# sebasv/lp

Hardware: AMD Instinct MI355X
Metric: IPM iterations/sec, dense 4096x8192 fp64 LP (higher is better)
Workload: dtype f64; 1 GPU; C3: random dense planted LP m=4096 n=8192 fp64, one independent LP per GPU (seed = rank), reference default options, A resident in HBM; m=4096, n=8192

## Files before the change

### lp_amd/csrc/kernels_adat.hip

```cpp
#include "gemm_tile.hpp"

namespace lpipm {

__device__ __forceinline__ int xcd_remap(int b, int n) {
    const int xcd = b & 7, q = n >> 3, r = n & 7;
    return (xcd < r ? xcd * (q + 1) : r * (q + 1) + (xcd - r) * q) + (b >> 3);
}

typedef unsigned int u4v __attribute__((ext_vector_type(4)));
typedef unsigned int u2v __attribute__((ext_vector_type(2)));
__device__ __forceinline__ __amdgpu_buffer_rsrc_t make_rsrc(const void* base, unsigned bytes) {
    return __builtin_amdgcn_make_buffer_rsrc(const_cast<void*>(base), 0, (int)bytes, 0x00020000);
}
__device__ __forceinline__ d2 buf_load_d2(__amdgpu_buffer_rsrc_t r, unsigned voff, unsigned soff) {
    return __builtin_bit_cast(d2, __builtin_amdgcn_raw_buffer_load_b128(r, (int)voff, (int)soff, 0));
}
__device__ __forceinline__ double buf_load_d(__amdgpu_buffer_rsrc_t r, unsigned voff, unsigned soff) {
    return __builtin_bit_cast(double, __builtin_amdgcn_raw_buffer_load_b64(r, (int)voff, (int)soff, 0));
}
__device__ __forceinline__ void buf_store_d(__amdgpu_buffer_rsrc_t r, unsigned voff, unsigned soff, double v) {
    __builtin_amdgcn_raw_buffer_store_b64(__builtin_bit_cast(u2v, v), r, (int)voff, (int)soff, 0);
}
template <int AUX>
__device__ __forceinline__ void buf_store_d_aux(__amdgpu_buffer_rsrc_t r, unsigned voff, unsigned soff, double v) {
    __builtin_amdgcn_raw_buffer_store_b64(__builtin_bit_cast(u2v, v), r, (int)voff, (int)soff, AUX);
}
template <int AUX>
__device__ __forceinline__ void buf_store_d2_aux(__amdgpu_buffer_rsrc_t r, unsigned voff, unsigned soff, d2 v) {
    __builtin_amdgcn_raw_buffer_store_b128(__builtin_bit_cast(u4v, v), r, (int)voff, (int)soff, AUX);
}
template <int AUX>
__device__ __forceinline__ d2 buf_load_d2_aux(__amdgpu_buffer_rsrc_t r, unsigned voff, unsigned soff) {
    return __builtin_bit_cast(d2, __builtin_amdgcn_raw_buffer_load_b128(r, (int)voff, (int)soff, AUX));
}

__device__ __forceinline__ int diag_pattern(int wr, int wc) {
    const int d = 2 * wc - 4 * wr;
    return d < 0 ? 0 : (d == 0 ? 1 : (d == 2 ? 2 : 3));
}
__device__ __forceinline__ void wave_part(int wave, int& wr, int& wc) {
    wr = (0x4B >> wave) & 1;
    wc = (0x7E84 >> (2 * wave)) & 3;
}
__device__ __forceinline__ constexpr int diag_group(int mi, int nj) {
    return nj > mi ? 1 : (2 + nj > mi ? 2 : 3);
}

template <typename F> __device__ __forceinline__ void diag_dispatch(int pat, F&& f) {
    if (pat == 0) f.template operator()<0>();
    else if (pat == 1) f.template operator()<1>();
    else if (pat == 2) f.template operator()<2>();
    else f.template operator()<3>();
}

template <int PAT = 0, typename FL, typename TC>
__device__ __forceinline__ void tile_pass_w8(double (*ldsA)[TILE][LDS_STRIDE], double (*ldsB)[TILE][LDS_STRIDE],
                                             __amdgpu_buffer_rsrc_t Pr, unsigned p64, __amdgpu_buffer_rsrc_t Qr, unsigned q64,
                                             __amdgpu_buffer_rsrc_t Sr, unsigned offP, unsigned offQ, unsigned offS,
                                             int kb, int ke, d4 (&acc)[4][2],
                                             int srow, int scol, int wr, int wc, int fr, int fq, int kc, FL&& flush,
                                             TC&& touch) {
    d2 sa[2], sb[2], sv;
    auto gload = [&](int kt) {
        const unsigned ko = (unsigned)kt * (unsigned)(BK * sizeof(double));
        sv = buf_load_d2(Sr, offS, ko);
        sa[0] = buf_load_d2(Pr, offP, ko);
        sa[1] = buf_load_d2(Pr, offP, ko + p64);
        sb[0] = buf_load_d2(Qr, offQ, ko);
        sb[1] = buf_load_d2(Qr, offQ, ko + q64);
    };
    auto lstore = [&](int buf) {
#pragma unroll
        for (int r = 0; r < 2; ++r) *(d2*)&ldsA[buf][srow + 64 * r][lds_wcol(srow, scol)] = sa[r];
#pragma unroll
        for (int r = 0; r < 2; ++r) *(d2*)&ldsB[buf][srow + 64 * r][lds_wcol(srow, scol)] = sb[r] * sv;
    };
    auto mfma_ktile = [&](int cur) {
        if constexpr (PAT < 3) {
#pragma unroll
            for (int round = 0; round < 2; ++round) {
                d2 a[4] = {}, b[2] = {};
                if (round == 0) __builtin_amdgcn_s_setprio(0);
#pragma unroll
                for (int mi = 0; mi < 4; ++mi)
                    if (diag_group(mi, 0) > PAT) a[mi] = *(const d2*)&ldsA[cur][wr * 64 + mi * 16 + fr][round * 8 + lds_rq(fr, fq)];
#pragma unroll
                for (int nj = 0; nj < 2; ++nj)
                    if (diag_group(3, nj) > PAT) b[nj] = *(const d2*)&ldsB[cur][wc * 32 + nj * 16 + fr][round * 8 + lds_rq(fr, fq)];
#pragma unroll
                for (int t = 0; t < 2; ++t)
#pragma unroll
                    for (int mi = 0; mi < 4; ++mi)
#pragma unroll
                        for (int nj = 0; nj < 2; ++nj)
                            if (diag_group(mi, nj) > PAT)
                                acc[mi][nj] = __builtin_amdgcn_mfma_f64_16x16x4f64(a[mi][t], b[nj][t], acc[mi][nj], 0, 0, 0);
            }
        }
        __builtin_amdgcn_s_setprio(2);
    };
    gload(kb);
    lstore(0);
    __syncthreads();
    int cur = 0, kt = kb;
    bool first = true;
    while (kt < ke) {
        int ce = ke;
        if (kc > 0) { const int e = (kt / kc + 1) * kc; ce = e < ke ? e : ke; }
        for (; kt < ce - 1; ++kt) {
            gload(kt + 1);
            mfma_ktile(cur);
            lstore(cur ^ 1);
            __syncthreads();
            cur ^= 1;
        }
        const bool more = ce < ke;
        unsigned pf0 = 0, pf1 = 0;
        touch(first, pf0, pf1);
        if (more) gload(ce);
        mfma_ktile(cur);
        if (more) lstore(cur ^ 1);
        asm volatile("" :: "v"(pf0), "v"(pf1));
        flush(first, !more);
        if (more) acc_clear(acc);
        first = false;
        __syncthreads();
        cur ^= 1;
        kt = ce;
    }
    __builtin_amdgcn_s_setprio(0);
}

struct Round2K {
    const double* A; long long lda;
    const double* s;
    double* C; long long ldc;
    int KT;
    int ntiles;
    const int2* tile_list;
    int diag_pad_from;
    double* ws;
    int nwg;
    unsigned int* sk_claim;
    int kc;
    int sk;
    double* C2;
    BatchK bk;
    long long astride;
};
__device__ __forceinline__ Round2K batch_shift(const Round2K& p0) {
    Round2K p = p0;
    p.A = (const double*)((const char*)p0.A + batch_lp(p0.bk) * p0.astride);
    p.s = batch_ptr(p0.s, p0.bk);
    p.C = batch_ptr(p0.C, p0.bk); p.ws = batch_ptr(p0.ws, p0.bk); p.sk_claim = batch_ptr(p0.sk_claim, p0.bk);
    p.C2 = batch_ptr(p0.C2, p0.bk);
    return p;
}
__global__ __launch_bounds__(512) __attribute__((amdgpu_waves_per_eu(4, 4))) void gemm_nt_streamk_w8_kernel(const Round2K p0) {
    if (batch_done(p0.bk)) return;
    const Round2K p = batch_shift(p0);
    __shared__ __attribute__((aligned(16))) double ldsA[2][TILE][LDS_STRIDE];
    __shared__ __attribute__((aligned(16))) double ldsB[2][TILE][LDS_STRIDE];
    const int tid = threadIdx.x, lane = tid & 63, wave = __builtin_amdgcn_readfirstlane(tid >> 6);
    int wr, wc;
    wave_part(wave, wr, wc);
    const int fr = lane & 15, fq = lane >> 4;
    const int srow = tid >> 3, scol = (tid & 7) * 2;
    const int g = p.bk.xcd_major ? (int)blockIdx.y : xcd_remap(blockIdx.x, gridDim.x);
    const int KT = p.KT;
    const int ntiles_dp = (p.ntiles / p.nwg) * p.nwg;
    const unsigned rowC = (unsigned)(p.ldc * (long long)sizeof(double));
    const unsigned offC = (unsigned)(wr * 64 + fq) * rowC + (unsigned)((wc * 32 + fr) * sizeof(double));
    auto c_rsrc = [&](int ti, int tj) { return make_rsrc(p.C + (long long)(ti * TILE) * p.ldc + tj * TILE, (unsigned)TILE * rowC); };
    auto store_tile = [&](const d4 (&acc)[4][2], int ti, int tj) {
        double* cb = p.C + (long long)(ti * TILE + wr * 64 + fq) * p.ldc + (tj * TILE + wc * 32 + fr);
        tile_store<4, 2>(cb, p.ldc, acc, 1.0, 0.0, p.diag_pad_from >= 0 && ti == tj, ti * TILE + wr * 64 + fq,
                         p.diag_pad_from, fr, fq, wc * 32 - wr * 64);
    };
    auto add_tile = [&](const d4 (&acc)[4][2], int ti, int tj, bool final_copy) {
        const __amdgpu_buffer_rsrc_t cr = c_rsrc(ti, tj);
        const __amdgpu_buffer_rsrc_t cr2 = make_rsrc((final_copy ? p.C2 : p.C) + (long long)(ti * TILE) * p.ldc + tj * TILE, (unsigned)TILE * rowC);
#pragma unroll
        for (int h = 0; h < 2; ++h) {
            double cv[2][4][2];
#pragma unroll
            for (int m2 = 0; m2 < 2; ++m2)
#pragma unroll
                for (int r = 0; r < 4; ++r)
#pragma unroll
                    for (int nj = 0; nj < 2; ++nj)
                        cv[m2][r][nj] = buf_load_d(cr, offC, (unsigned)((2 * h + m2) * 16 + 4 * r) * rowC + nj * 128);
#pragma unroll
            for (int m2 = 0; m2 < 2; ++m2)
#pragma unroll
                for (int r = 0; r < 4; ++r)
#pragma unroll
                    for (int nj = 0; nj < 2; ++nj)
                    {
                        const double v = cv[m2][r][nj] + acc[2 * h + m2][nj][r];
                        buf_store_d(cr, offC, (unsigned)((2 * h + m2) * 16 + 4 * r) * rowC + nj * 128, v);
                        if (final_copy) buf_store_d(cr2, offC, (unsigned)((2 * h + m2) * 16 + 4 * r) * rowC + nj * 128, v);
                    }
        }
    };
    auto touch_tile = [&](int ti, int tj, unsigned& pf0, unsigned& pf1) {
        const __amdgpu_buffer_rsrc_t cr = c_rsrc(ti, tj);
        const unsigned off = (unsigned)(wr * 64 + lane) * rowC + (unsigned)(wc * 32 * sizeof(double));
        pf0 = __builtin_amdgcn_raw_buffer_load_b32(cr, (int)off, 0, 0);
        pf1 = __builtin_amdgcn_raw_buffer_load_b32(cr, (int)off, 128, 0);
    };
    const unsigned rowA = (unsigned)(p.lda * (long long)sizeof(double));
    const unsigned offP = (unsigned)srow * rowA + (unsigned)(scol * sizeof(double));
    const unsigned offS = (unsigned)(scol * sizeof(double));
    const unsigned p64 = 64u * rowA;
    auto a_rsrc = [&](int t) { return make_rsrc(p.A + (long long)(t * TILE) * p.lda, (unsigned)TILE * rowA); };
    const __amdgpu_buffer_rsrc_t Sr = make_rsrc(p.s, (unsigned)KT * (unsigned)(BK * sizeof(double)));
    for (int tile = g; tile < ntiles_dp; tile += p.nwg) {
        const int ti = p.tile_list[tile].x, tj = p.tile_list[tile].y;
        d4 acc[4][2];
        acc_clear(acc);
        tile_pass_w8(ldsA, ldsB, a_rsrc(ti), p64, a_rsrc(tj), p64, Sr, offP, offP, offS, 0, KT, acc, srow, scol, wr, wc, fr, fq,
                            p.kc, [&](bool first, bool last) {
                                if (first) store_tile(acc, ti, tj); else add_tile(acc, ti, tj, last && p.C2 != nullptr);
                            },
                            [&](bool first, unsigned& pf0, unsigned& pf1) { if (!first) touch_tile(ti, tj, pf0, pf1); });
    }
    if (ntiles_dp == p.ntiles) return;
    __shared__ int s_claim;
    const int ch_tiles = p.sk;
    const int cpt = (KT + ch_tiles - 1) / ch_tiles;
    const int nchunks = (p.ntiles - ntiles_dp) * cpt;
    for (;;) {
        if (tid == 0) s_claim = (int)atomicAdd(p.sk_claim, 1u);
        __syncthreads();
        const int ch = __builtin_amdgcn_readfirstlane(s_claim);
        __syncthreads();
        if (ch >= nchunks) break;
        const int nrem = p.ntiles - ntiles_dp;
        const int q = ch / nrem, rt = ch - q * nrem;
        const int kb = q * ch_tiles, ke = kb + ch_tiles < KT ? kb + ch_tiles : KT;
        const int ti = p.tile_list[ntiles_dp + rt].x, tj = p.tile_list[ntiles_dp + rt].y;
        d4 acc[4][2];
        acc_clear(acc);
        tile_pass_w8(ldsA, ldsB, a_rsrc(ti), p64, a_rsrc(tj), p64, Sr, offP, offP, offS, kb, ke, acc, srow, scol, wr, wc, fr, fq,
                            0, [&](bool, bool) {
            if (cpt == 1) { store_tile(acc, ti, tj); return; }
            const __amdgpu_buffer_rsrc_t wr_ = make_rsrc(p.ws + ((long long)rt * cpt + q) * (TILE * TILE), (unsigned)(TILE * TILE * sizeof(double)));
            const unsigned offW = (unsigned)(((wr * 64 + fq) * TILE + wc * 32 + fr) * sizeof(double));
#pragma unroll
            for (int mi = 0; mi < 4; ++mi)
#pragma unroll
                for (int r = 0; r < 4; ++r)
#pragma unroll
                    for (int nj = 0; nj < 2; ++nj)
                        buf_store_d(wr_, offW, (unsigned)(((mi * 16 + 4 * r) * TILE + nj * 16) * sizeof(double)), acc[mi][nj][r]);
        }, [](bool, unsigned&, unsigned&) {});
    }
}

constexpr int FIX_SPLIT = 16;
__global__ __launch_bounds__(256) void gemm_nt_fixup_kernel(const Round2K p0) {
    if (batch_done(p0.bk)) return;
    const Round2K p = batch_shift(p0);
    const int ntiles_dp = (p.ntiles / p.nwg) * p.nwg;
    const int bx = p.bk.xcd_major ? (int)blockIdx.y : (int)blockIdx.x;
    const int rt = bx / FIX_SPLIT, part = bx % FIX_SPLIT;
    const int cpt = (p.KT + p.sk - 1) / p.sk;
    const int ti = p.tile_list[ntiles_dp + rt].x, tj = p.tile_list[ntiles_dp + rt].y;
    constexpr int PER = TILE * TILE / FIX_SPLIT;
    const double* slab0 = p.ws + (long long)rt * cpt * (TILE * TILE);
    for (int e = part * PER + threadIdx.x * 2; e < (part + 1) * PER; e += 512) {
        d2 sum = *(const d2*)(slab0 + e);
        for (int q = 1; q < cpt; ++q) sum += *(const d2*)(slab0 + (long long)q * (TILE * TILE) + e);
        const int r = e / TILE, c = e - r * TILE;
        const int row = ti * TILE + r, col = tj * TILE + c;
        double* cp = p.C + (long long)row * p.ldc + col;
        d2 v = sum;
        if (p.diag_pad_from >= 0) {
            if (row == col && row >= p.diag_pad_from) v[0] = 1.0;
            if (row == col + 1 && row >= p.diag_pad_from) v[1] = 1.0;
        }
        *(d2*)cp = v;
        if (p.C2) *(d2*)(p.C2 + (long long)row * p.ldc + col) = v;
    }
}

constexpr int AUX_SC1 = 16;
struct UnitsK {
    const double* A; long long lda;
    const double* s;
    double* C; long long ldc;
    double* C2;
    int KT, kc, cpt;
    int nbig, ks;
    int ntiles;
    const int2* tile_list;
    const int2* unit_list;
    int nunits, upc;
    int diag_pad_from;
    double* slabs;
    unsigned int* tile_cnt;
    unsigned int* grp_cnt;
    int grp_w;
    BatchK bk;
    long long astride;
};
template <bool GRP>
__global__ __launch_bounds__(512) __attribute__((amdgpu_waves_per_eu(4, 4))) void gemm_nt_units_kernel(const UnitsK p0) {
    if (batch_done(p0.bk)) return;
    UnitsK p = p0;
    p.A = (const double*)((const char*)p0.A + batch_lp(p0.bk) * p0.astride);
    p.s = batch_ptr(p0.s, p0.bk); p.C = batch_ptr(p0.C, p0.bk); p.C2 = batch_ptr(p0.C2, p0.bk);
    p.slabs = batch_ptr(p0.slabs, p0.bk); p.tile_cnt = batch_ptr(p0.tile_cnt, p0.bk); p.grp_cnt = batch_ptr(p0.grp_cnt, p0.bk);
    __shared__ __attribute__((aligned(16))) double ldsA[2][TILE][LDS_STRIDE];
    __shared__ __attribute__((aligned(16))) double ldsB[2][TILE][LDS_STRIDE];
    __shared__ unsigned int s_old;
    const int tid = threadIdx.x, lane = tid & 63, wave = __builtin_amdgcn_readfirstlane(tid >> 6);
    int wr, wc;
    wave_part(wave, wr, wc);
    const int fr = lane & 15, fq = lane >> 4;
    const int srow = tid >> 3, scol = (tid & 7) * 2;
    const int b = p.bk.xcd_major ? (int)blockIdx.y : (int)blockIdx.x;
    const int2 un = p.unit_list[b];
    const int tile = un.x, q0 = un.y;
    if (tile < 0) return;
    const int q1 = q0 + p.upc < p.cpt ? q0 + p.upc : p.cpt;
    const int2 tc = p.tile_list[tile];
    const int ti = tc.x, tj = tc.y;
    const int KT = p.KT;
    const unsigned rowA = (unsigned)(p.lda * (long long)sizeof(double));
    const unsigned offP = (unsigned)srow * rowA + (unsigned)(scol * sizeof(double));
    const unsigned offS = (unsigned)(scol * sizeof(double));
    const unsigned p64 = 64u * rowA;
    const __amdgpu_buffer_rsrc_t Pr = make_rsrc(p.A + (long long)(ti * TILE) * p.lda, (unsigned)TILE * rowA);
    const __amdgpu_buffer_rsrc_t Qr = make_rsrc(p.A + (long long)(tj * TILE) * p.lda, (unsigned)TILE * rowA);
    const __amdgpu_buffer_rsrc_t Sr = make_rsrc(p.s, (unsigned)KT * (unsigned)(BK * sizeof(double)));
    constexpr unsigned SLAB_BYTES = (unsigned)(TILE * TILE * sizeof(double));
    const __amdgpu_buffer_rsrc_t Wr = make_rsrc(p.slabs + (long long)tile * p.cpt * (TILE * TILE), (unsigned)p.cpt * SLAB_BYTES);
    d4 acc[4][2];
    acc_clear(acc);
    auto chunk_begin = [&](int q) { const int b0 = q <= p.nbig ? q * p.kc : p.nbig * p.kc + (q - p.nbig) * p.ks; return b0 < KT ? b0 : KT; };
    const int kb = chunk_begin(q0), ke = chunk_begin(q1);
    const int dpat = ti == tj ? diag_pattern(wr, wc) : 0;
    if (p.cpt == 1) {
        diag_dispatch(dpat, [&]<int PAT>() {
            tile_pass_w8<PAT>(ldsA, ldsB, Pr, p64, Qr, p64, Sr, offP, offP, offS, 0, KT, acc, srow, scol, wr, wc, fr, fq, 0,
                                    [&](bool, bool) {}, [](bool, unsigned&, unsigned&) {});
        });
        const unsigned rowC = (unsigned)(p.ldc * (long long)sizeof(double));
        const unsigned offC = (unsigned)(wr * 64 + fq) * rowC + (unsigned)((wc * 32 + fr) * sizeof(double));
        const __amdgpu_buffer_rsrc_t cr = make_rsrc(p.C + (long long)(ti * TILE) * p.ldc + tj * TILE, (unsigned)TILE * rowC);
        const __amdgpu_buffer_rsrc_t cr2 = make_rsrc((p.C2 ? p.C2 : p.C) + (long long)(ti * TILE) * p.ldc + tj * TILE, (unsigned)TILE * rowC);
        const bool pad = p.diag_pad_from >= 0 && ti == tj;
        const int row0 = ti * TILE + wr * 64 + fq, dd = wc * 32 - wr * 64;
#pragma unroll
        for (int mi = 0; mi < 4; ++mi)
#pragma unroll
            for (int r = 0; r < 4; ++r)
#pragma unroll
                for (int nj = 0; nj < 2; ++nj) {
                    double v = acc[mi][nj][r];
                    if (pad && (mi - nj) * 16 + fq + 4 * r - fr == dd && row0 + mi * 16 + 4 * r >= p.diag_pad_from) v = 1.0;
                    const unsigned so = (unsigned)(mi * 16 + 4 * r) * rowC + nj * 128;
                    buf_store_d_aux<GRP ? AUX_SC1 : 0>(cr, offC, so, v);
                    if (p.C2) buf_store_d_aux<0>(cr2, offC, so, v);
                }
    } else {
        int q = q0;
        const unsigned offW = (unsigned)(((wr * 64 + fq) * TILE + wc * 32 + fr) * sizeof(double));
        diag_dispatch(dpat, [&]<int PAT>() {
        tile_pass_w8<PAT>(ldsA, ldsB, Pr, p64, Qr, p64, Sr, offP, offP, offS, kb, ke, acc, srow, scol, wr, wc, fr, fq, p.kc,
                           [&](bool, bool) {
                               const unsigned sb = (unsigned)q * SLAB_BYTES;
#pragma unroll
                               for (int mi = 0; mi < 4; ++mi)
#pragma unroll
                                   for (int r = 0; r < 4; ++r)
#pragma unroll
                                       for (int nj = 0; nj < 2; ++nj)
                                           buf_store_d_aux<AUX_SC1>(Wr, offW, sb + (unsigned)(((mi * 16 + 4 * r) * TILE + nj * 16) * sizeof(double)),
                                                                    acc[mi][nj][r]);
                               ++q;
                           },
                           [](bool, unsigned&, unsigned&) {});
        });
        asm volatile("s_waitcnt vmcnt(0)" ::: "memory");
        __syncthreads();
        if (tid == 0) s_old = __hip_atomic_fetch_add(p.tile_cnt + tile, (unsigned)(q1 - q0), __ATOMIC_RELAXED, __HIP_MEMORY_SCOPE_AGENT);
        __syncthreads();
        if ((int)s_old + (q1 - q0) != p.cpt) return;
        if (tid == 0) {
            __builtin_amdgcn_fence(__ATOMIC_ACQUIRE, "agent");
            asm volatile("s_waitcnt vmcnt(0)" ::: "memory");
            if (!GRP) __hip_atomic_store(p.tile_cnt + tile, 0u, __ATOMIC_RELAXED, __HIP_MEMORY_SCOPE_AGENT);
        }
        __syncthreads();
        const unsigned rowC = (unsigned)(p.ldc * (long long)sizeof(double));
        const __amdgpu_buffer_rsrc_t cr = make_rsrc(p.C + (long long)(ti * TILE) * p.ldc + tj * TILE, (unsigned)TILE * rowC);
        const __amdgpu_buffer_rsrc_t cr2 = make_rsrc((p.C2 ? p.C2 : p.C) + (long long)(ti * TILE) * p.ldc + tj * TILE, (unsigned)TILE * rowC);
        const unsigned voff = (unsigned)tid * 16u;
        const int cpt = p.cpt;
        for (int i = 0; i < 16; i += 2) {
            d2 sum[2];
#pragma unroll
            for (int a = 0; a < 2; ++a)
                sum[a] = buf_load_d2_aux<AUX_SC1>(Wr, voff, (unsigned)(i + a) * 8192u);
            for (int qb = 1; qb < cpt; qb += 4) {
                d2 v[2][4];
#pragma unroll
                for (int j = 0; j < 4; ++j)
#pragma unroll
                    for (int a = 0; a < 2; ++a)
                        if (qb + j < cpt)
                            v[a][j] = buf_load_d2_aux<AUX_SC1>(Wr, voff, (unsigned)(qb + j) * SLAB_BYTES + (unsigned)(i + a) * 8192u);
#pragma unroll
                for (int j = 0; j < 4; ++j)
#pragma unroll
                    for (int a = 0; a < 2; ++a)
                        if (qb + j < cpt) sum[a] += v[a][j];
            }
#pragma unroll
            for (int a = 0; a < 2; ++a) {
                const int e = tid * 2 + (i + a) * 1024;
                const int r = e >> 7, c = e & 127;
                const int row = ti * TILE + r, col = tj * TILE + c;
                d2 v = sum[a];
                if (p.diag_pad_from >= 0 && ti == tj) {
                    if (row == col && row >= p.diag_pad_from) v[0] = 1.0;
                    if (row == col + 1 && row >= p.diag_pad_from) v[1] = 1.0;
                }
                const unsigned co = (unsigned)r * rowC + (unsigned)(c * sizeof(double));
                buf_store_d2_aux<GRP ? AUX_SC1 : 0>(cr, co, 0u, v);
                if (p.C2) buf_store_d2_aux<0>(cr2, co, 0u, v);
            }
        }
    }
    if (GRP) {
        asm volatile("s_waitcnt vmcnt(0)" ::: "memory");
        __syncthreads();
        if (tid == 0) (void)__hip_atomic_fetch_add(p.grp_cnt + tj / p.grp_w, 1u, __ATOMIC_RELAXED, __HIP_MEMORY_SCOPE_AGENT);
    }
}

__global__ __launch_bounds__(64) void wait_count_kernel(const unsigned int* cnt, unsigned int target, const int* done,
                                                        unsigned int* timeout) {
    if (threadIdx.x != 0) return;
    if (done && __hip_atomic_load(done, __ATOMIC_RELAXED, __HIP_MEMORY_SCOPE_AGENT) != 0) return;
    for (unsigned int spins = 0; spins < (1u << 21); ++spins) {
        if (__hip_atomic_load(cnt, __ATOMIC_RELAXED, __HIP_MEMORY_SCOPE_AGENT) >= target) return;
        __builtin_amdgcn_s_sleep(16);
    }
    __hip_atomic_store(timeout, 1u, __ATOMIC_RELAXED, __HIP_MEMORY_SCOPE_AGENT);
}

static int canonical_chunk(int KT) { return KT <= 64 ? 8 : (KT <= 256 ? 16 : 64); }
static int round2_unit(int KT) {
    const int kc = canonical_chunk(KT);
    return KT <= 256 ? kc : (kc < 16 ? kc : 16);
}
static int round2_cpt(int KT) {
    if (KT <= canonical_chunk(KT)) return 1;
    const int u = round2_unit(KT);
    return (KT + u - 1) / u;
}
static int round2_nwg(int ntiles, int KT, int num_cu) {
    const int cpt = round2_cpt(KT);
    const long long units = (long long)ntiles * cpt;
    long long nwg = 2LL * num_cu;
    if (nwg > units) nwg = units;
    if (nwg < 1) nwg = 1;
    return (int)nwg;
}
static size_t round2_slabs(int ntiles, int KT, int nwg) {
    const int cpt = round2_cpt(KT);
    const int nrem = ntiles - (ntiles / nwg) * nwg;
    return cpt > 1 ? (size_t)nrem * cpt : 0;
}

static int units_chunking(int K, int* kc_out, int* nbig_out, int* ks_out) {
    const int KT = K / BK, kc = canonical_chunk(KT);
    int nbig, ks, cpt;
    if (KT <= kc) { nbig = 1; ks = kc; cpt = 1; }
    else if (KT <= 256 || kc < 32) { ks = kc; cpt = (KT + kc - 1) / kc; nbig = cpt; }
    else {
        nbig = KT / kc - 1;
        ks = kc / 4;
        cpt = nbig + (KT - nbig * kc + ks - 1) / ks;
    }
    *kc_out = kc; *nbig_out = nbig; *ks_out = ks;
    return cpt;
}
constexpr int UNITS_MAX_CPT = 256;

AdatPlan plan_adat(int mp, int npa, int count, int num_cu, int world, int units_env) {
    AdatPlan a;
    const int nt = mp / TILE;
    a.ntiles = nt * (nt + 1) / 2;
    if (count == 1) a.nwg = round2_nwg(a.ntiles, npa / BK, num_cu);
    else if ((long long)count * a.ntiles >= 2LL * num_cu) {
        a.nwg = 2 * num_cu / count;
        if (a.nwg < 1) a.nwg = 1;
        if (a.nwg > a.ntiles) a.nwg = a.ntiles;
    } else {
        a.nwg = round2_nwg(a.ntiles, npa / BK, num_cu / count);
        if (a.nwg < a.ntiles) a.nwg = a.ntiles;
    }
    a.slabs = round2_slabs(a.ntiles, npa / BK, a.nwg);
    int kc, nbig, ks;
    a.cpt = units_chunking(npa, &kc, &nbig, &ks);
    const bool units_fit = a.cpt <= UNITS_MAX_CPT;
    a.units = units_env != 0 && units_fit && (size_t)a.ntiles * a.cpt * TILE * TILE * sizeof(double) <= ((size_t)4 << 30) &&
               (count > 1 || units_env == 2 || a.cpt == 1 || a.ntiles <= 16 || a.ntiles * a.cpt >= 256);
    if (count == 1 && world > 1 && units_env != 0 && units_fit && nt <= 64 * POTRF_OUTER &&
        (size_t)a.ntiles * a.cpt * TILE * TILE * sizeof(double) <= ((size_t)32 << 30)) a.units = true;
    a.grouped = count == 1 && world > 1 && a.units && nt >= 1 && nt <= 64 * POTRF_OUTER;
    a.upc = count == 1 ? 1 : (a.cpt < 2 ? a.cpt : 2);
    if (a.cpt != nbig) a.upc = 1;
    if (a.units && a.slabs < (size_t)a.ntiles * a.cpt) a.slabs = (size_t)a.ntiles * a.cpt;
    return a;
}

void adat_take(AdatRes& r, const AdatPlan& plan, Arena& ar) {
    r.claim = ar.take<unsigned int>(1);
    r.counter_bytes = (size_t)round_up(((size_t)plan.ntiles + 64) * sizeof(unsigned int), 16);
    r.counters = (unsigned int*)ar.take<uint4>(r.counter_bytes / 16);
    r.group_words = r.counters + plan.ntiles;
    r.wait_timeout = ar.take<unsigned int>(4);
    r.slabs = ar.take<double>(plan.slabs * TILE * TILE);
}

static std::vector<int2> tile_order(int nt) {
    std::vector<int2> v;
    v.reserve((size_t)nt * (nt + 1) / 2);
    const int ns = (nt + 7) / 8;
    auto emit = [&](int SI, int SJ) {
        for (int ti = SI * 8; ti < nt && ti < SI * 8 + 8; ++ti)
            for (int tj = SJ * 8; tj < SJ * 8 + 8 && tj <= ti; ++tj) v.push_back(make_int2(ti, tj));
    };
    for (int SI = 0; SI < ns; ++SI)
        for (int SJ = 0; SJ < SI; ++SJ) emit(SI, SJ);
    for (int SI = 0; SI < ns; ++SI) emit(SI, SI);
    return v;
}
static std::vector<int2> tile_order_grouped(int nt, std::vector<int>& off, std::vector<int>& cnt) {
    std::vector<int2> v;
    for (int g = 0; g * POTRF_OUTER < nt; ++g) {
        off.push_back((int)v.size());
        const int c0 = g * POTRF_OUTER, c1 = c0 + POTRF_OUTER < nt ? c0 + POTRF_OUTER : nt;
        for (int ti = c0; ti < nt; ++ti)
            for (int tj = c0; tj < c1 && tj <= ti; ++tj) v.push_back(make_int2(ti, tj));
        cnt.push_back((int)v.size() - off.back());
    }
    return v;
}
static void deal_units(int first, int nt, int cpt, int upc, std::vector<int2>& out) {
    std::vector<int> own[8];
    const int full = nt / 512 * 512, rest = nt - full;
    for (int i = 0; i < full; ++i) own[(i % 512) / 64].push_back(first + i);
    for (int x = 0; x < 8; ++x)
        for (int i = full + (int)((long long)rest * x / 8); i < full + (int)((long long)rest * (x + 1) / 8); ++i) own[x].push_back(first + i);
    size_t longest = 0;
    for (int x = 0; x < 8; ++x) longest = own[x].size() > longest ? own[x].size() : longest;
    const int nq = (cpt + upc - 1) / upc;
    for (int q = 0; q < nq; ++q)
        for (size_t i = 0; i < longest; ++i)
            for (int x = 0; x < 8; ++x)
                out.push_back(i < own[x].size() ? make_int2(own[x][i], q * upc) : make_int2(-1, 0));
}

void adat_lists_destroy(AdatRes& r) {
    if (r.tiles) (void)hipFree(r.tiles);
    r.tiles = r.tiles_grouped = r.units = r.units_grouped = nullptr;
    r.nunits = r.nunits_grouped = 0;
    r.list_bytes = 0;
    r.group_first.clear(); r.group_ntiles.clear();
}
hipError_t adat_lists_create(AdatRes& r, const AdatPlan& plan, int mp, int count, hipStream_t st) {
    adat_lists_destroy(r);
    r.counters_dirty = true;
    const int nt = mp / TILE;
    const std::vector<int2> order = tile_order(nt);
    std::vector<int2> units, grouped, units_grp;
    if (plan.units) {
        if (count == 1) deal_units(0, plan.ntiles, plan.cpt, plan.upc, units);
        else
            for (int q = 0; q < plan.cpt; q += plan.upc)
                for (int t = 0; t < plan.ntiles; ++t) units.push_back(make_int2(t, q));
    }
    if (plan.grouped) {
        grouped = tile_order_grouped(nt, r.group_first, r.group_ntiles);
        for (size_t g = 0; g < r.group_ntiles.size(); ++g) deal_units(r.group_first[g], r.group_ntiles[g], plan.cpt, 1, units_grp);
    }
    r.nunits = (int)units.size(); r.nunits_grouped = (int)units_grp.size();
    r.list_bytes = (order.size() + grouped.size() + units.size() + units_grp.size() + 1) * sizeof(int2);
    hipError_t e = hipMalloc((void**)&r.tiles, r.list_bytes);
    if (e != hipSuccess) { r.tiles = nullptr; r.list_bytes = 0; return e; }
    r.tiles_grouped = r.tiles + order.size();
    r.units = r.tiles_grouped + grouped.size();
    r.units_grouped = r.units + units.size();
    auto put = [&](int2* dst, const std::vector<int2>& v) {
        return v.empty() ? hipSuccess : hipMemcpyAsync(dst, v.data(), v.size() * sizeof(int2), hipMemcpyHostToDevice, st);
    };
    if ((e = put(r.tiles, order)) != hipSuccess || (e = put(r.tiles_grouped, grouped)) != hipSuccess ||
        (e = put(r.units, units)) != hipSuccess || (e = put(r.units_grouped, units_grp)) != hipSuccess) return e;
    return hipStreamSynchronize(st);
}

static hipError_t clear_words(unsigned int* w, size_t bytes, const Batch& bt, hipStream_t st) {
    char* p = (char*)w + (size_t)bt.first * (size_t)bt.stride;
    return bt.count == 1 ? hipMemsetAsync(p, 0, bytes, st) : hipMemset2DAsync(p, (size_t)bt.stride, 0, bytes, (size_t)bt.count, st);
}

static hipError_t launch_units(const AdatPlan& plan, AdatRes& r, const AdatLaunch& a, bool signal_groups, hipStream_t st,
                               bool second_copy, hipEvent_t armed) {
    hipError_t e;
    if ((signal_groups || (plan.cpt > 1 && r.counters_dirty)) && (e = clear_words(r.counters, r.counter_bytes, a.batch, st)) != hipSuccess) return e;
    r.counters_dirty = signal_groups;
    if (armed && (e = hipEventRecord(armed, st)) != hipSuccess) return e;
    const int nunits = signal_groups ? r.nunits_grouped : r.nunits;
    if (plan.ntiles <= 0 || nunits <= 0 || a.K <= 0) return hipSuccess;
    UnitsK k{};
    k.A = a.A; k.lda = a.lda; k.s = a.dinv; k.C = a.M; k.ldc = a.ldm; k.C2 = second_copy ? a.M2 : nullptr;
    k.KT = a.K / BK;
    k.cpt = units_chunking(a.K, &k.kc, &k.nbig, &k.ks);
    if (k.cpt == 1) k.kc = 0;
    k.upc = signal_groups ? 1 : plan.upc;
    if (k.cpt != plan.cpt || (k.upc > 1 && k.nbig != k.cpt)) return hipErrorInvalidValue;
    k.ntiles = plan.ntiles; k.nunits = nunits;
    k.tile_list = signal_groups ? r.tiles_grouped : r.tiles; k.unit_list = signal_groups ? r.units_grouped : r.units;
    k.diag_pad_from = a.diag_pad_from; k.slabs = r.slabs; k.tile_cnt = r.counters;
    k.grp_cnt = signal_groups ? r.group_words : nullptr; k.grp_w = POTRF_OUTER; k.bk = batch_k(a.batch);
    k.astride = a.shared_a ? 0 : k.bk.stride;
    const int B = a.batch.count;
    const bool xm = B >= 8 && B % 8 == 0;
    k.bk.xcd_major = xm ? 1 : 0;
    const dim3 grid = xm ? dim3(8, nunits, B / 8) : dim3(nunits, 1, B);
    if (signal_groups) hipLaunchKernelGGL(gemm_nt_units_kernel<true>, grid, dim3(512), 0, st, k);
    else               hipLaunchKernelGGL(gemm_nt_units_kernel<false>, grid, dim3(512), 0, st, k);
    return hipGetLastError();
}

static hipError_t launch_round2(const AdatPlan& plan, AdatRes& r, const AdatLaunch& a, hipStream_t st, bool second_copy) {
    Round2K k;
    k.A = a.A; k.lda = a.lda; k.s = a.dinv; k.C = a.M; k.ldc = a.ldm; k.KT = a.K / BK;
    k.ntiles = plan.ntiles; k.tile_list = r.tiles; k.diag_pad_from = a.diag_pad_from;
    k.ws = r.slabs; k.nwg = plan.nwg; k.sk_claim = r.claim; k.C2 = second_copy ? a.M2 : nullptr;
    k.bk = batch_k(a.batch);
    k.astride = a.shared_a ? 0 : k.bk.stride;
    const int B = a.batch.count;
    if (plan.ntiles <= 0 || k.KT <= 0) return hipSuccess;
    k.kc = canonical_chunk(k.KT);
    if (k.KT <= k.kc) k.kc = 0;
    k.sk = k.kc == 0 ? k.KT : round2_unit(k.KT);
    const int cpt = round2_cpt(k.KT);
    const int nrem = plan.ntiles - (plan.ntiles / plan.nwg) * plan.nwg;
    if (nrem > 0) {
        hipError_t em = clear_words(r.claim, sizeof(unsigned int), a.batch, st);
        if (em != hipSuccess) return em;
    }
    const bool xm = B >= 8 && B % 8 == 0;
    k.bk.xcd_major = xm ? 1 : 0;
    const dim3 grid = xm ? dim3(8, plan.nwg, B / 8) : dim3(plan.nwg, 1, B);
    hipLaunchKernelGGL(gemm_nt_streamk_w8_kernel, grid, dim3(512), 0, st, k);
    hipError_t e = hipGetLastError();
    if (e != hipSuccess) return e;
    if (nrem > 0 && cpt > 1) {
        hipLaunchKernelGGL(gemm_nt_fixup_kernel, xm ? dim3(8, nrem * FIX_SPLIT, B / 8) : dim3(nrem * FIX_SPLIT, 1, B), dim3(256), 0,
                           st, k);
        e = hipGetLastError();
    }
    return e;
}

hipError_t launch_adat(const AdatPlan& plan, AdatRes& r, const AdatLaunch& a, bool signal_groups, hipStream_t st,
                       bool* second_copy, hipEvent_t armed) {
    if (!a.A || !a.dinv || !a.M || !r.tiles || !r.claim) return hipErrorInvalidValue;
    if (a.lda >= (1 << 22) || a.ldm >= (1 << 22)) return hipErrorInvalidValue;
    if (signal_groups && !(plan.units && plan.grouped)) return hipErrorInvalidValue;
    const bool second = a.M2 != nullptr && plan.cpt > 1 && !signal_groups;
    if (second_copy) *second_copy = second;
    return plan.units ? launch_units(plan, r, a, signal_groups, st, second, armed) : launch_round2(plan, r, a, st, second);
}

hipError_t launch_wait_count(const unsigned int* cnt, unsigned int target, const int* done, unsigned int* timeout, hipStream_t st) {
    hipLaunchKernelGGL(wait_count_kernel, dim3(1), dim3(64), 0, st, cnt, target, done, timeout);
    return hipGetLastError();
}

}
```

Measured before the change: 269.5 iterations/s.

## Load ADAT GEMM tiles directly into LDS via buffer-load-to-LDS DMA with swizzled layout

Replaces the register-staged global-to-LDS copy in the A·D·Aᵀ units kernel with buffer_load ... lds direct transfers into a new XOR-swizzled LDS image that also holds the diagonal scaling vector. The scaling by D moves from the load stage into the MFMA stage as a multiply on the B fragments. The k-loop is restructured into a two-round, double-buffered schedule with one barrier per k-tile. The aim is to remove VGPR staging and LDS store instructions and to overlap DMA with MFMA, at the cost of extra VALU multiplies and a different bank-conflict pattern.

```diff
diff --git a/lp_amd/csrc/adat_lds_image.hpp b/lp_amd/csrc/adat_lds_image.hpp
--- /dev/null
+++ b/lp_amd/csrc/adat_lds_image.hpp
@@ -0,0 +1,26 @@
+#pragma once
+
+namespace lpipm {
+namespace adat_image {
+
+constexpr int ROW_BYTES = 128;
+constexpr int BLOCKS = 8;
+constexpr int PIECE_ROWS = 8;
+constexpr int PANEL_BYTES = 128 * ROW_BYTES;
+constexpr int D_BYTES = 128;
+constexpr int PANELS_OFF = 256;
+constexpr int BUF_BYTES = 2 * PANEL_BYTES;
+constexpr int FLAG_OFF = PANELS_OFF + 2 * BUF_BYTES;
+constexpr int LDS_BYTES = FLAG_OFF + 16;
+constexpr int panel_base(int buf, int panel) { return PANELS_OFF + buf * BUF_BYTES + panel * PANEL_BYTES; }
+constexpr int d_base(int buf) { return buf * D_BYTES; }
+
+constexpr int swz(int row) { return (row >> 1) & 7; }
+constexpr int src_block(int row, int pos) { return pos ^ swz(row); }
+constexpr int read_offset(int row, int kb) { return row * ROW_BYTES + ((kb ^ swz(row)) << 4); }
+constexpr int piece_row(int row0, int lane) { return row0 + (lane >> 3); }
+constexpr int piece_lds_offset(int row0, int lane) { return row0 * ROW_BYTES + lane * 16; }
+constexpr int piece_src_offset(int row0, int lane) { return src_block(piece_row(row0, lane), lane & 7) << 4; }
+
+}
+}
diff --git a/lp_amd/csrc/kernels_adat.hip b/lp_amd/csrc/kernels_adat.hip
--- a/lp_amd/csrc/kernels_adat.hip
+++ b/lp_amd/csrc/kernels_adat.hip
@@ -1,4 +1,5 @@
 #include "gemm_tile.hpp"
+#include "adat_lds_image.hpp"
 
 namespace lpipm {
 
@@ -131,6 +132,85 @@
     __builtin_amdgcn_s_setprio(0);
 }
 
+__device__ __forceinline__ void lds_dma16(__amdgpu_buffer_rsrc_t r, char* dst, unsigned voff, unsigned soff) {
+    __builtin_amdgcn_raw_ptr_buffer_load_lds(r, (__attribute__((address_space(3))) void*)dst, 16, (int)voff, (int)soff, 0, 0);
+}
+__device__ __forceinline__ int fresh(int v) { asm volatile("" : "+v"(v)); return v; }
+template <int PAT = 0, typename FL>
+__device__ __forceinline__ void tile_pass_dma(char* lds, __amdgpu_buffer_rsrc_t Pr, __amdgpu_buffer_rsrc_t Qr, unsigned r64,
+                                              __amdgpu_buffer_rsrc_t Sr, unsigned offP, int kb, int ke, d4 (&acc)[4][2],
+                                              int tid, int wave, int wr, int wc, int kc, FL&& flush) {
+    namespace im = adat_image;
+    const bool dlane = wave == 0 && (tid & 63) < 8;
+    auto dma = [&](int kt, int bo) {
+        const unsigned ko = (unsigned)kt * (unsigned)im::ROW_BYTES;
+        char* pb = lds + im::PANELS_OFF + bo + wave * (im::PIECE_ROWS * im::ROW_BYTES);
+        lds_dma16(Pr, pb, offP, ko);
+        lds_dma16(Pr, pb + 64 * im::ROW_BYTES, offP, ko + r64);
+        lds_dma16(Qr, pb + im::PANEL_BYTES, offP, ko);
+        lds_dma16(Qr, pb + im::PANEL_BYTES + 64 * im::ROW_BYTES, offP, ko + r64);
+        if (dlane) lds_dma16(Sr, lds + (bo >> 8), offP, ko);
+    };
+    const int aoff = im::read_offset(wr * 64 + (tid & 15), (tid & 63) >> 4);
+    const int bdelta = im::PANEL_BYTES + (wc * 32 - wr * 64) * im::ROW_BYTES;
+    auto rd = [&](int bo, int round, d2 (&a)[4], d2 (&b)[2], d2& dv) {
+        if constexpr (PAT < 3) {
+            const int ra = (fresh(aoff) ^ (round << 6)) + (im::PANELS_OFF + bo);
+#pragma unroll
+            for (int mi = 0; mi < 4; ++mi)
+                if (diag_group(mi, 0) > PAT) a[mi] = *(const d2*)(lds + (ra + mi * 16 * im::ROW_BYTES));
+#pragma unroll
+            for (int nj = 0; nj < 2; ++nj)
+                if (diag_group(3, nj) > PAT) b[nj] = *(const d2*)(lds + (ra + bdelta + nj * 16 * im::ROW_BYTES));
+            dv = *(const d2*)(lds + ((fresh(tid) & 48) + (bo >> 8) + round * 64));
+        }
+    };
+    auto mfma_round = [&](const d2 (&a)[4], d2 (&b)[2], const d2& dv) {
+        if constexpr (PAT < 3) {
+#pragma unroll
+            for (int nj = 0; nj < 2; ++nj)
+                if (diag_group(3, nj) > PAT) b[nj] = b[nj] * dv;
+#pragma unroll
+            for (int t = 0; t < 2; ++t)
+#pragma unroll
+                for (int mi = 0; mi < 4; ++mi)
+#pragma unroll
+                    for (int nj = 0; nj < 2; ++nj)
+                        if (diag_group(mi, nj) > PAT)
+                            acc[mi][nj] = __builtin_amdgcn_mfma_f64_16x16x4f64(a[mi][t], b[nj][t], acc[mi][nj], 0, 0, 0);
+        }
+    };
+    d2 a0[4] = {}, b0[2] = {}, a1[4] = {}, b1[2] = {}, dv0 = {}, dv1 = {};
+    static_assert(im::BUF_BYTES >> 8 == im::D_BYTES && im::PANELS_OFF % 256 == 0, "d_base(buf) == (buf * BUF_BYTES) >> 8");
+    int cur = 0;
+    auto ktile = [&](int kt) {
+        rd(cur, 1, a1, b1, dv1);
+        mfma_round(a0, b0, dv0);
+        __builtin_amdgcn_s_setprio(2);
+        __syncthreads();
+        if (kt + 2 < ke) dma(kt + 2, cur);
+        cur ^= im::BUF_BYTES;
+        if (kt + 1 < ke) rd(cur, 0, a0, b0, dv0);
+        __builtin_amdgcn_s_setprio(0);
+        mfma_round(a1, b1, dv1);
+    };
+    dma(kb, 0);
+    __syncthreads();
+    if (kb + 1 < ke) dma(kb + 1, im::BUF_BYTES);
+    rd(0, 0, a0, b0, dv0);
+    int kt = kb;
+    bool first = true;
+    while (kt < ke) {
+        int ce = ke;
+        if (kc > 0) { const int e = (kt / kc + 1) * kc; ce = e < ke ? e : ke; }
+        for (; kt < ce; ++kt) ktile(kt);
+        const bool more = ce < ke;
+        flush(first, !more);
+        if (more) acc_clear(acc);
+        first = false;
+    }
+}
+
 struct Round2K {
     const double* A; long long lda;
     const double* s;
@@ -312,14 +392,12 @@
     p.A = (const double*)((const char*)p0.A + batch_lp(p0.bk) * p0.astride);
     p.s = batch_ptr(p0.s, p0.bk); p.C = batch_ptr(p0.C, p0.bk); p.C2 = batch_ptr(p0.C2, p0.bk);
     p.slabs = batch_ptr(p0.slabs, p0.bk); p.tile_cnt = batch_ptr(p0.tile_cnt, p0.bk); p.grp_cnt = batch_ptr(p0.grp_cnt, p0.bk);
-    __shared__ __attribute__((aligned(16))) double ldsA[2][TILE][LDS_STRIDE];
-    __shared__ __attribute__((aligned(16))) double ldsB[2][TILE][LDS_STRIDE];
-    __shared__ unsigned int s_old;
-    const int tid = threadIdx.x, lane = tid & 63, wave = __builtin_amdgcn_readfirstlane(tid >> 6);
+    __shared__ __attribute__((aligned(256))) char lds[adat_image::LDS_BYTES];
+    unsigned int& s_old = *(unsigned int*)(lds + adat_image::FLAG_OFF);
+    const int tid0 = threadIdx.x, wave = __builtin_amdgcn_readfirstlane(tid0 >> 6);
     int wr, wc;
     wave_part(wave, wr, wc);
-    const int fr = lane & 15, fq = lane >> 4;
-    const int srow = tid >> 3, scol = (tid & 7) * 2;
+    const int srow = tid0 >> 3;
     const int b = p.bk.xcd_major ? (int)blockIdx.y : (int)blockIdx.x;
     const int2 un = p.unit_list[b];
     const int tile = un.x, q0 = un.y;
@@ -329,8 +407,7 @@
     const int ti = tc.x, tj = tc.y;
     const int KT = p.KT;
     const unsigned rowA = (unsigned)(p.lda * (long long)sizeof(double));
-    const unsigned offP = (unsigned)srow * rowA + (unsigned)(scol * sizeof(double));
-    const unsigned offS = (unsigned)(scol * sizeof(double));
+    const unsigned offP = (unsigned)srow * rowA + (unsigned)(adat_image::src_block(srow, tid0 & 7) << 4);
     const unsigned p64 = 64u * rowA;
     const __amdgpu_buffer_rsrc_t Pr = make_rsrc(p.A + (long long)(ti * TILE) * p.lda, (unsigned)TILE * rowA);
     const __amdgpu_buffer_rsrc_t Qr = make_rsrc(p.A + (long long)(tj * TILE) * p.lda, (unsigned)TILE * rowA);
@@ -344,9 +421,9 @@
     const int dpat = ti == tj ? diag_pattern(wr, wc) : 0;
     if (p.cpt == 1) {
         diag_dispatch(dpat, [&]<int PAT>() {
-            tile_pass_w8<PAT>(ldsA, ldsB, Pr, p64, Qr, p64, Sr, offP, offP, offS, 0, KT, acc, srow, scol, wr, wc, fr, fq, 0,
-                                    [&](bool, bool) {}, [](bool, unsigned&, unsigned&) {});
+            tile_pass_dma<PAT>(lds, Pr, Qr, p64, Sr, offP, 0, KT, acc, tid0, wave, wr, wc, 0, [&](bool, bool) {});
         });
+        const int tid = fresh(tid0), fr = tid & 15, fq = (tid & 63) >> 4;
         const unsigned rowC = (unsigned)(p.ldc * (long long)sizeof(double));
         const unsigned offC = (unsigned)(wr * 64 + fq) * rowC + (unsigned)((wc * 32 + fr) * sizeof(double));
         const __amdgpu_buffer_rsrc_t cr = make_rsrc(p.C + (long long)(ti * TILE) * p.ldc + tj * TILE, (unsigned)TILE * rowC);
@@ -367,10 +444,11 @@
                 }
     } else {
         int q = q0;
-        const unsigned offW = (unsigned)(((wr * 64 + fq) * TILE + wc * 32 + fr) * sizeof(double));
         diag_dispatch(dpat, [&]<int PAT>() {
-        tile_pass_w8<PAT>(ldsA, ldsB, Pr, p64, Qr, p64, Sr, offP, offP, offS, kb, ke, acc, srow, scol, wr, wc, fr, fq, p.kc,
+        tile_pass_dma<PAT>(lds, Pr, Qr, p64, Sr, offP, kb, ke, acc, tid0, wave, wr, wc, p.kc,
                            [&](bool, bool) {
+                               const int tf = fresh(tid0), fr = tf & 15, fq = (tf & 63) >> 4;
+                               const unsigned offW = (unsigned)(((wr * 64 + fq) * TILE + wc * 32 + fr) * sizeof(double));
                                const unsigned sb = (unsigned)q * SLAB_BYTES;
 #pragma unroll
                                for (int mi = 0; mi < 4; ++mi)
@@ -381,9 +459,9 @@
                                            buf_store_d_aux<AUX_SC1>(Wr, offW, sb + (unsigned)(((mi * 16 + 4 * r) * TILE + nj * 16) * sizeof(double)),
                                                                     acc[mi][nj][r]);
                                ++q;
-                           },
-                           [](bool, unsigned&, unsigned&) {});
+                           });
         });
+        const int tid = fresh(tid0);
         asm volatile("s_waitcnt vmcnt(0)" ::: "memory");
         __syncthreads();
         if (tid == 0) s_old = __hip_atomic_fetch_add(p.tile_cnt + tile, (unsigned)(q1 - q0), __ATOMIC_RELAXED, __HIP_MEMORY_SCOPE_AGENT);
@@ -438,7 +516,7 @@
     if (GRP) {
         asm volatile("s_waitcnt vmcnt(0)" ::: "memory");
         __syncthreads();
-        if (tid == 0) (void)__hip_atomic_fetch_add(p.grp_cnt + tj / p.grp_w, 1u, __ATOMIC_RELAXED, __HIP_MEMORY_SCOPE_AGENT);
+        if (tid0 == 0) (void)__hip_atomic_fetch_add(p.grp_cnt + tj / p.grp_w, 1u, __ATOMIC_RELAXED, __HIP_MEMORY_SCOPE_AGENT);
     }
 }
 
```

New measurement: 271.2 iterations/s, median of 6. About the same (+0.6%).
